# YuvalNirkin/hyperseg

Measured on AMD Instinct MI355X. Metric: frames/sec @ bs=1 HyperSeg-M 1024x512, higher is better.
Workload: dtype f32 storage and accumulation; level-4 inverted residual products as 3-term f16 splits (f32-class: 1.3e-7 of sum|a||b|; exact_f32 beside it)

## Files before the change

hyperseg_amd/_hip.py:

```python
import ctypes as C
import os

import torch

_LIB_PATH = os.environ.get('HS_HIP_LIB') or os.path.join(os.path.dirname(os.path.abspath(__file__)), 'lib',
                                                         'libhyperseg_hip.so')

ACT_NONE, ACT_RELU, ACT_RELU6, ACT_SWISH = 0, 1, 2, 3
PAD_MODES = {'zeros': 0, 'reflect': 1, 'replicate': 2, 'circular': 3}
PREV_NONE, PREV_SAME, PREV_BILINEAR = 0, 1, 2

_STATUS = {-1: 'bad argument', -2: 'feature map does not tile into the weight grid (H % fh or W % fw != 0)',
           -3: 'unsupported shape', -4: 'tile does not fit the LDS'}


class HipLibraryError(RuntimeError):
    pass


class StageInputC(C.Structure):
    _fields_ = [('skip', C.c_void_p), ('prev', C.c_void_p),
                ('batch', C.c_int32), ('H', C.c_int32), ('W', C.c_int32),
                ('c_skip', C.c_int32), ('c_prev', C.c_int32),
                ('Hp', C.c_int32), ('Wp', C.c_int32),
# ... 113 lines not shown
        'hs_patch_conv_plain_bwd_w': ([i32, vp, vp, i32, i32, i32, i32, i32, i32, i32, i32, i32, i32, i32, vp, i64, vp], C.c_int),
        'hs_depthwise_conv_fwd': ([vp, i32, i32, i32, i32, vp, i32, i32, i32, i32, i32, i32, vp, vp, i32, vp, vp, vp, vp, vp], C.c_int),
        'hs_pointwise_conv_fwd': ([vp, i32, i32, i32, vp, i32, vp, vp, vp, i32, vp, vp, vp], C.c_int),
        'hs_affine_act_fwd': ([vp, i32, i32, i32, vp, vp, i32, vp, vp, vp], C.c_int),
        'hs_patch_conv_bn_fwd': ([i32, vp, vp, vp, vp, vp, vp, C.c_float, C.c_float, i32, vp, vp, vp, vp, i64, i32, i32, i32, i32, i32, i32, i32, vp, vp], C.c_int),
        'hs_patch_conv_bn_bwd_w': ([i32, vp, vp, vp, vp, vp, vp, i32, i32, i32, i32, i32, i32, i32, i32, vp, i64, vp], C.c_int),
        'hs_bootstrap_mean_of_batch_fwd': ([vp, i32, i32, i32, C.c_float, vp, vp, vp, vp], C.c_int),
        'hs_bootstrap_mean_of_batch_bwd': ([vp, i32, i32, vp, vp, vp, vp], C.c_int),
        'hs_adam_blocks': ([vp, i32], C.c_int64),
        'hs_adam_step': ([vp, vp, vp, vp, vp, i32, vp, C.c_float, C.c_double, C.c_double, C.c_float, C.c_float, i32, i32, vp, vp], C.c_int),
        'hs_depthwise_pool_blocks': ([i32, i32], C.c_int),
        'hs_depthwise_conv_se_fwd': ([vp, i32, i32, i32, i32, vp, i32, i32, i32, i32, i32, i32, vp, vp, i32, vp, vp, vp, C.POINTER(SeTailC), vp], C.c_int),
        'hs_mbconv_expand_dw_se_fwd': ([vp, i32, i32, i32, i32, vp, i32, vp, vp, vp, i32, i32, i32, i32, i32, i32, vp, vp, vp, C.POINTER(SeTailC), vp], C.c_int),
        'hs_se_tail_workspace': ([i32, i32, i32, i32, i64], C.c_int64),
        'hs_se_tail_tails': ([i32, i32, i32, i64], C.c_int),
        'hs_mbconv_se_workgroups': ([i32, i32, i32, i32, i32, i32], C.c_int64),
        'hs_stem_conv_fwd': ([vp, i32, i32, i32, i32, vp, i32, i32, i32, i32, i32, vp, vp, vp, vp], C.c_int),
        'hs_mbconv_tiles': ([i32, i32, i32, i32], C.c_int),
        'hs_stem_dw_fwd': ([vp, i32, i32, i32, vp, i32, vp, vp, i32, i32, i32, i32, vp, i32, i32, i32, vp, vp, vp, vp, vp], C.c_int),
        'hs_mbconv_expand_dw_fwd': ([vp, i32, i32, i32, i32, vp, i32, vp, vp, vp, i32, i32, i32, i32, i32, i32, vp, vp, vp, vp, vp], C.c_int),
        'hs_se_gate_fwd': ([vp, i32, i32, i32, C.c_float, vp, vp, i32, vp, vp, vp, vp, vp, i32, vp, vp, vp], C.c_int),
        'hs_gemm_split_kp': ([i32], C.c_int),
        'hs_gemm_split_fwd': ([vp, vp, vp, vp, vp, i32, vp, vp, i32, i32, i32, i32, i32, vp], C.c_int),
        'hs_gemm_split_conv2x2_fwd': ([vp, vp, vp, vp, i32, vp, vp, i32, i32, i32, i32, i32, i32, vp], C.c_int),
        'hs_gemm_split_up2_fwd': ([vp, vp, vp, vp, i32, vp, i32, i32, i32, i32, i32, i32, vp], C.c_int),
        'hs_pooled_shift_fwd': ([vp, i32, C.c_float, vp, vp, vp, i32, i32, vp], C.c_int),
    }
    for name, (argtypes, restype) in sig.items():
        fn = getattr(lib, name)
        fn.argtypes, fn.restype = argtypes, restype
    if lib.hs_version() != 1:
        raise HipLibraryError(f'ABI mismatch: library reports version {lib.hs_version()}, binding expects 1')
    return lib


lib = _load()
EXPORTS = ['hs_version', 'hs_build_info', 'hs_signal2weights_fwd', 'hs_signal2weights_multi_fwd', 'hs_s2w_pack_floats', 'hs_s2w_pack_fwd', 'hs_bank_pack_fwd', 'hs_bn_fold_fwd',
           'hs_patch_conv_fwd', 'hs_patch_conv_s2w_fwd', 'hs_k1_chain_workspace', 'hs_k1_chain_fwd', 'hs_decoder_chain_workspace', 'hs_decoder_chain_fwd', 'hs_meta_conv_fwd', 'hs_meta_conv_bwd', 'hs_patch_conv_gen_fwd', 'hs_patch_ir_fwd', 'hs_patch_ir_v0_fwd', 'hs_patch_ir_v0_ws_fwd', 'hs_patch_ir_v0_workspace', 'hs_patch_ir_route', 'hs_ir_tile_map', 'hs_upsample_bilinear_fwd', 'hs_upsample_argmax_fwd',
           'hs_stage_input_fwd', 'hs_depthwise_conv_fwd', 'hs_depthwise_pool_blocks', 'hs_stem_conv_fwd', 'hs_stem_dw_fwd', 'hs_mbconv_tiles', 'hs_mbconv_expand_dw_fwd', 'hs_se_gate_fwd', 'hs_depthwise_conv_se_fwd', 'hs_mbconv_expand_dw_se_fwd', 'hs_se_tail_workspace', 'hs_se_tail_tails', 'hs_mbconv_se_workgroups', 'hs_pointwise_conv_fwd', 'hs_affine_act_fwd', 'hs_gemm_split_kp', 'hs_gemm_split_fwd', 'hs_gemm_split_conv2x2_fwd', 'hs_gemm_split_up2_fwd', 'hs_pooled_shift_fwd', 'hs_patch_conv_bwd_input',
           'hs_patch_conv_bwd_weight', 'hs_halo_tiles_fwd', 'hs_halo_tiles_bwd', 'hs_tile_interior_fwd', 'hs_tile_interior_bwd', 'hs_dw_tiles_fwd', 'hs_dw_tiles_bwd_in', 'hs_dw_tiles_bwd_w',
           'hs_s2w_train_fwd', 'hs_s2w_train_workspace', 'hs_s2w_train_bwd', 'hs_cross_entropy_fwd', 'hs_cross_entropy_bwd', 'hs_cross_entropy_typed_fwd', 'hs_cross_entropy_typed_bwd', 'hs_bootstrapped_ce_fwd', 'hs_bootstrapped_ce_bwd', 'hs_bootstrap_mean_workspace', 'hs_bootstrap_mean_fwd', 'hs_bootstrap_mean_bwd', 'hs_bootstrap_mean_batched_fwd', 'hs_bootstrap_mean_batched_bwd', 'hs_bn_train_workspace', 'hs_bn_train_stats_fwd', 'hs_dw_tiles_bn_fwd', 'hs_dw_tiles_bn_bwd_w', 'hs_patch_conv_bn_fwd', 'hs_patch_conv_bn_bwd_w', 'hs_adam_blocks', 'hs_adam_step', 'hs_bootstrap_mean_of_batch_fwd', 'hs_bootstrap_mean_of_batch_bwd', 'hs_upsample_bilinear_bwd', 'hs_upsample_bilinear_typed_bwd', 'hs_upsample_bilinear_bf16_fwd', 'hs_stage_input_typed_fwd', 'hs_bank_unpack_fwd', 'hs_bn_act_train_fwd',
           'hs_bn_act_train_bwd', 'hs_dw_tiles_bn_bwd_in_partials', 'hs_dw_tiles_bn_bwd_in', 'hs_bn_act_train_bwd_apply', 'hs_patch_conv_plain_fwd', 'hs_patch_conv_plain_bwd_in', 'hs_patch_conv_plain_bwd_w']


def check(status, what):
    if status == 0:
        return
    if status < 0:
        raise HipLibraryError(f'{what}: {_STATUS.get(status, status)}')
    raise HipLibraryError(f'{what}: HIP launch failed with hipError_t {status}')


def dev_ptr(t, name='tensor', dtype=torch.float32):
    if t is None:
        return None
    if not isinstance(t, torch.Tensor):
        raise TypeError(f'{name} must be a torch.Tensor')
    if not t.is_cuda:
        raise HipLibraryError(f'{name} is on {t.device}: the HyperSeg decoder path runs on an MI355X only '
                              '(hyperseg_amd has no CPU fallback)')
    if t.dtype != dtype:
        raise HipLibraryError(f'{name} must be {dtype}, got {t.dtype}')
# ... 25 lines not shown
```

hyperseg_amd/csrc/hs_gemm_split.hip:

```cpp
#include "hs_common.h"
#include <type_traits>

namespace hs {

using half8 = __attribute__((ext_vector_type(8))) _Float16;
using gs_f32x4 = __attribute__((ext_vector_type(4))) float;

__device__ __forceinline__ int gs_exp_of(float m) { return min(max(__float_as_int(m) >> 23, 27), 254); }
__device__ __forceinline__ float gs_scale_of(int eb) { return __int_as_float((268 - eb) << 23); }
__device__ __forceinline__ float gs_inv_scale_of(int eb) { return __int_as_float((eb - 14) << 23); }

struct GemmSplitArgs {
    const _Float16* __restrict__ wf;
    const float* __restrict__ w_inv;
    const float* __restrict__ gate; const float* __restrict__ x;
    const float* shift;
    const float* residual;
    float* y;
    int M, K, KST, N, act;
    int conv_wo;
    float* pool_partial;
    int up2_wo;
};

#ifndef HS_GS_NARROW_MAX_WG
#define HS_GS_NARROW_MAX_WG 128
#endif

#ifndef HS_GS_TALL_MIN_WG
#define HS_GS_TALL_MIN_WG 257
#endif

template <int KS, int NWV, bool FAST, int NS, int MT, int NCH, bool PATCH>
__global__ __launch_bounds__(64 * NWV)
void gemm_split_kernel(GemmSplitArgs a) {
    extern __shared__ __attribute__((aligned(16))) float gs_red[];
    constexpr int nthr = 64 * NWV, nwv = NWV;
    constexpr int NP = 16 * NS, NR = 16 * MT, NE = NR * NP;
    const int tid = threadIdx.x, lane = tid & 63, wave = tid >> 6;
    const int lrow = lane & 15, kg = lane >> 4;
    const int n0 = blockIdx.x * NP, r0 = blockIdx.y * MT, b = blockIdx.z;
    const float* __restrict__ xb = a.x + (size_t)b * a.K * a.N;
    const float* __restrict__ gb = a.gate ? a.gate + (size_t)b * a.K : nullptr;
    float* yb = a.y + (size_t)b * a.M * a.N * (a.up2_wo > 0 ? 4 : 1);
    const float* rb = a.residual ? a.residual + (size_t)b * a.M * a.N : nullptr;
    const int rt_max = (a.M + 15) >> 4;

    using gs_f32x2 = __attribute__((ext_vector_type(2))) float;
    const int ncol0 = min(n0 + NS * lrow, a.N - 1), ncol1 = min(n0 + NS * lrow + 1, a.N - 1);
    float xv[NCH][NS][KS][8];
    if constexpr (PATCH) {
        const int oy = ncol0 / a.conv_wo, ox = ncol0 - oy * a.conv_wo;
        const float* __restrict__ win = xb + (size_t)(2 * oy) * (2 * a.conv_wo) + 2 * ox;
        const int cmax = (a.K >> 2) - 1;
#pragma unroll
        for (int c = 0; c < NCH; ++c)
#pragma unroll
            for (int s = 0; s < KS; ++s)
#pragma unroll
                for (int q = 0; q < 4; ++q) {
                    const int ch = min((((wave * NCH + c) * KS + s) * 32 + 8 * kg) / 4 + (q >> 1), cmax);
                    const float* src = win + (size_t)ch * (4 * a.N) + (q & 1) * (2 * a.conv_wo);
                    if constexpr (NS == 1) {
                        const gs_f32x2 v = *reinterpret_cast<const gs_f32x2*>(src);
                        xv[c][0][s][2 * q] = v[0]; xv[c][0][s][2 * q + 1] = v[1];
                    } else {
                        const gs_f32x4 v = *reinterpret_cast<const gs_f32x4*>(src);
                        xv[c][0][s][2 * q] = v[0]; xv[c][0][s][2 * q + 1] = v[1];
                        xv[c][1][s][2 * q] = v[2]; xv[c][1][s][2 * q + 1] = v[3];
                    }
                }
    } else {
#pragma unroll
        for (int c = 0; c < NCH; ++c)
#pragma unroll
            for (int s = 0; s < KS; ++s)
#pragma unroll
                for (int j = 0; j < 8; ++j) {
                    const int k = ((wave * NCH + c) * KS + s) * 32 + 8 * kg + j;
                    const int kc = min(k, a.K - 1);
                    if constexpr (NS == 1) {
                        xv[c][0][s][j] = xb[(size_t)kc * a.N + ncol0];
                    } else if constexpr (FAST) {
                        const gs_f32x2 v = *reinterpret_cast<const gs_f32x2*>(xb + (size_t)kc * a.N + ncol0);
                        xv[c][0][s][j] = v[0]; xv[c][1][s][j] = v[1];
                    } else {
                        xv[c][0][s][j] = xb[(size_t)kc * a.N + ncol0]; xv[c][1][s][j] = xb[(size_t)kc * a.N + ncol1];
                    }
                }
    }
    constexpr int NG = PATCH ? 1 : NCH;
    float gv[NG][KS][8];
    if constexpr (!PATCH) {
#pragma unroll
        for (int c = 0; c < NCH; ++c)
#pragma unroll
            for (int s = 0; s < KS; ++s) {
                const int k0 = ((wave * NCH + c) * KS + s) * 32 + 8 * kg;
                if constexpr (FAST) {
                    const float* gp = gb ? gb + min(k0, a.K - 8) : a.w_inv;
                    const gs_f32x4 g0 = *reinterpret_cast<const gs_f32x4*>(gp), g1 = *reinterpret_cast<const gs_f32x4*>(gp + 4);
#pragma unroll
                    for (int j = 0; j < 4; ++j) { gv[c][s][j] = g0[j]; gv[c][s][4 + j] = g1[j]; }
                } else {
#pragma unroll
                    for (int j = 0; j < 8; ++j) gv[c][s][j] = gb ? gb[min(k0 + j, a.K - 1)] : 1.0f;
                }
            }
    }
    half8 ah[2][KS], al[2][KS];
    auto load_a = [&](int q) {
        const int rt = min(r0 + q % MT, rt_max - 1);
#pragma unroll
        for (int s = 0; s < KS; ++s) {
            const _Float16* blk = a.wf + ((size_t)(rt * a.KST + (wave * NCH + q / MT) * KS + s) * 2) * 512 + lane * 8;
            ah[q & 1][s] = *reinterpret_cast<const half8*>(blk);
            al[q & 1][s] = *reinterpret_cast<const half8*>(blk + 512);
        }
    };
    load_a(0);
    constexpr int TE = (NE + nthr - 1) / nthr;
    float wi[TE], sh[TE], yo[TE];
    auto load_tail = [&]() {
#pragma unroll
        for (int i = 0; i < TE; ++i) {
            const int e = min(tid + i * nthr, NE - 1);
            const int row = min(16 * r0 + e / NP, a.M - 1), col = min(n0 + (e & (NP - 1)), a.N - 1);
            wi[i] = a.w_inv[min(16 * r0 + e / NP, 16 * rt_max - 1)];
            sh[i] = a.shift ? a.shift[row] : 0.0f;
            yo[i] = rb ? rb[(size_t)row * a.N + col] : 0.0f;
        }
    };
    constexpr bool LATE_TAIL = KS * NCH >= 3;
    if constexpr (!LATE_TAIL) load_tail();
    __builtin_amdgcn_sched_barrier(0);

    gs_f32x4 tot[MT][NS];
#pragma unroll
    for (int c = 0; c < NCH; ++c) {
        float invb[NS];
        half8 bh[NS][KS], bl[NS][KS];
#pragma unroll
        for (int t = 0; t < NS; ++t) {
            unsigned mx = 0;
#pragma unroll
            for (int s = 0; s < KS; ++s) {
                const int k0 = ((wave * NCH + c) * KS + s) * 32 + 8 * kg;
#pragma unroll
                for (int j = 0; j < 8; ++j) {
                    const float mk = (FAST || PATCH ? k0 : k0 + j) < a.K ? 1.0f : 0.0f;
                    float g = mk;
                    if constexpr (!PATCH) g = gb ? gv[c][s][j] * mk : mk;
                    xv[c][t][s][j] *= g;
                    mx = max(mx, __float_as_uint(xv[c][t][s][j]) & 0x7fffffffu);
                }
            }
            {
                auto r16 = __builtin_amdgcn_permlane16_swap(mx, mx, false, false);
                mx = max(r16[0], r16[1]);
                auto r32 = __builtin_amdgcn_permlane32_swap(mx, mx, false, false);
                mx = max(r32[0], r32[1]);
            }
            const int eb = gs_exp_of(__uint_as_float(mx));
            const float sc = gs_scale_of(eb);
            invb[t] = gs_inv_scale_of(eb);
#pragma unroll
            for (int s = 0; s < KS; ++s) {
                if constexpr (FAST || PATCH) {
                    unsigned hh[4], ll[4];
#pragma unroll
                    for (int j = 0; j < 4; ++j) {
                        asm("v_fma_mixlo_f16 %0, %2, %4, 0\n\t"
                            "v_fma_mixhi_f16 %0, %3, %4, 0\n\t"
                            "v_fma_mixlo_f16 %1, %2, %4, -%0 op_sel_hi:[0,0,1]\n\t"
                            "v_fma_mixhi_f16 %1, %3, %4, -%0 op_sel:[0,0,1] op_sel_hi:[0,0,1]"
// ... 114 lines not shown

static bool gemm_split_plan(int K, int& nwv, int& ks, int& nch) {
    const int steps = (K + 31) / 32;
    nwv = 2;
    while (nwv < 8 && nwv < steps) nwv *= 2;
    const int per = (steps + nwv - 1) / nwv;
    nch = per > 5 ? 2 : 1;
    ks = (steps + nwv * nch - 1) / (nwv * nch);
    return ks <= 5;
}

}

using namespace hs;

extern "C" int hs_gemm_split_kp(int32_t c_in) {
    int nwv, ks, nch;
    if (c_in <= 0 || !gemm_split_plan(c_in, nwv, ks, nch)) return HS_ERR_UNSUPPORTED;
    return nwv * nch * ks * 32;
}

static int launch_gemm_split_plain(const void* w_frag, const float* w_inv, const float* gate, const float* x, const float* shift,
                                   int32_t act, const float* residual, float* y, int32_t batch, int32_t c_out, int32_t c_in,
                                   int32_t kp, int32_t pixels, int up2_wo, void* stream) {
    if (!w_frag || !w_inv || !x || !y || batch <= 0 || c_out <= 0 || c_in <= 0 || pixels <= 0) return HS_ERR_BAD_ARG;
    if (act < 0 || act > 3) return HS_ERR_BAD_ARG;
    int nwv, ks, nch;
    if (!gemm_split_plan(c_in, nwv, ks, nch)) return HS_ERR_UNSUPPORTED;
    if (kp != nwv * nch * ks * 32 || (ks > 1 && nwv != 8)) return HS_ERR_BAD_ARG;
    if (batch > 65535 || (c_out + 31) / 32 > 65535) return HS_ERR_UNSUPPORTED;
    GemmSplitArgs a{(const _Float16*)w_frag, w_inv, gate, x, shift, residual, y, c_out, c_in, kp / 32, pixels, act, 0, nullptr, up2_wo};
    dim3 grid((pixels + 31) / 32, ((c_out + 15) / 16 + 1) / 2, batch);
    const size_t wgs = (size_t)grid.x * grid.y * grid.z;
    const bool narrow = wgs <= HS_GS_NARROW_MAX_WG && pixels > 16;
    const bool tall = wgs >= HS_GS_TALL_MIN_WG && c_out > 32;
    if (narrow) grid.x = (pixels + 15) / 16;
    if (tall) grid.y = ((c_out + 15) / 16 + 3) / 4;
    const size_t lds = (size_t)nwv * (narrow ? 512 : tall ? 2048 : 1024) * sizeof(float);
    hipStream_t s = (hipStream_t)stream;
    const bool fast = (c_in & 7) == 0 && (pixels & 1) == 0 && c_in >= 8;
#define HS_GS_(KSV, NWV, F) do { \
        if (narrow) hipLaunchKernelGGL((gemm_split_kernel<KSV, NWV, F, 1, 2, 1, false>), grid, dim3(64 * NWV), lds, s, a); \
        else if (tall) hipLaunchKernelGGL((gemm_split_kernel<KSV, NWV, F, 2, 4, 1, false>), grid, dim3(64 * NWV), lds, s, a); \
        else hipLaunchKernelGGL((gemm_split_kernel<KSV, NWV, F, 2, 2, 1, false>), grid, dim3(64 * NWV), lds, s, a); } while (0)
#define HS_GS(KSV, NWV) do { if (fast) HS_GS_(KSV, NWV, true); else HS_GS_(KSV, NWV, false); } while (0)
    if (nch == 2) {
        if (!fast || up2_wo > 0) return HS_ERR_UNSUPPORTED;
        grid.x = (pixels + 15) / 16; grid.y = ((c_out + 15) / 16 + 1) / 2;
        const size_t lds2 = (size_t)8 * 512 * sizeof(float);
#define HS_GS2(KSV) hipLaunchKernelGGL((gemm_split_kernel<KSV, 8, true, 1, 2, 2, false>), grid, dim3(512), lds2, s, a)
        switch (ks) { case 3: HS_GS2(3); break; case 4: HS_GS2(4); break; case 5: HS_GS2(5); break; default: return HS_ERR_UNSUPPORTED; }
#undef HS_GS2
        return launch_status();
    }
    switch (ks) {
        case 1: if (nwv == 2) HS_GS(1, 2); else if (nwv == 4) HS_GS(1, 4); else HS_GS(1, 8); break;
        case 2: HS_GS(2, 8); break;
        case 3: HS_GS(3, 8); break;
        case 4: HS_GS(4, 8); break;
        default: HS_GS(5, 8); break;
    }
#undef HS_GS
#undef HS_GS_
    return launch_status();
}

extern "C" int hs_gemm_split_fwd(const void* w_frag, const float* w_inv, const float* gate, const float* x,
                                 const float* shift, int32_t act, const float* residual, float* y,
                                 int32_t batch, int32_t c_out, int32_t c_in, int32_t kp, int32_t pixels, void* stream) {
    return launch_gemm_split_plain(w_frag, w_inv, gate, x, shift, act, residual, y, batch, c_out, c_in, kp, pixels, 0, stream);
}

extern "C" int hs_gemm_split_up2_fwd(const void* w_frag, const float* w_inv, const float* x, const float* shift, int32_t act,
                                     float* y, int32_t batch, int32_t c_out, int32_t c_in, int32_t kp, int32_t Ho, int32_t Wo,
                                     void* stream) {
    if (Ho <= 0 || Wo <= 0 || (((size_t)y) & 7) != 0) return HS_ERR_BAD_ARG;
    return launch_gemm_split_plain(w_frag, w_inv, nullptr, x, shift, act, nullptr, y, batch, c_out, c_in, kp, Ho * Wo, Wo, stream);
}

extern "C" int hs_pooled_shift_fwd(const float* partial, int32_t nblk, float inv_pixels, const float* wb, const float* shift,
                                   float* shift_out, int32_t rows, int32_t channels, void* stream) {
    if (!partial || !wb || !shift || !shift_out || nblk <= 0 || rows <= 0 || channels <= 0) return HS_ERR_BAD_ARG;
    if (channels > 8192) return HS_ERR_UNSUPPORTED;
    hipLaunchKernelGGL(pooled_shift_kernel, dim3((rows + 15) / 16), dim3(256), (size_t)channels * sizeof(float), (hipStream_t)stream,
                       partial, nblk, inv_pixels, wb, shift, shift_out, rows, channels);
    return launch_status();
}

extern "C" int hs_gemm_split_conv2x2_fwd(const void* w_frag, const float* w_inv, const float* x, const float* shift, int32_t act,
                                         float* y, float* pool_partial, int32_t batch, int32_t c_out, int32_t c_in, int32_t kp,
                                         int32_t Ho, int32_t Wo, void* stream) {
    if (!w_frag || !w_inv || !x || !y || batch <= 0 || c_out <= 0 || c_in <= 0 || Ho <= 0 || Wo <= 0) return HS_ERR_BAD_ARG;
    if (act < 0 || act > 3) return HS_ERR_BAD_ARG;
// ... 26 lines not shown
```

hyperseg_amd/functional.py:

```python
import ctypes as C
import functools
import os
import threading

import torch

from . import _hip
from ._hip import ACT_NONE, ACT_RELU, ACT_RELU6, PAD_MODES

BN_EPS_DEFAULT = 1e-5
S2W_TRAIN_MAX_LAYERS = 8
USE_SIDE_STREAM = os.environ.get('HS_SIDE_STREAM', '0') == '1'
PIPELINE_BANKS = os.environ.get('HS_SIDE_STREAM', '0') == '2'
COSCHEDULE_BANKS = os.environ.get('HS_COSCHEDULE_BANKS', '0') == '1'


def _round_up(n, m):
    return (n + m - 1) // m * m


def _device_of(a):
    if isinstance(a, torch.Tensor):
        return a.device
    if isinstance(a, (StageInput, BankRef, SignalRef)):
# ... 910 lines not shown
    m, k = w.shape
    kp = _hip.lib.hs_gemm_split_kp(k) if k <= max_k else -1
    if kp < 0:
        return None
    if row_scale is not None:
        w = w * row_scale.detach().float()[:, None]
    eb = (w.abs().amax(1).contiguous().view(torch.int32) >> 23).clamp(27, 254)
    one = torch.ones(m, device=w.device)
    ws = w * torch.ldexp(one, 141 - eb)[:, None]
    hi = ws.half()
    lo = (ws - hi.float()).half()
    rt = -(-m // 16)
    pad = (0, kp - k, 0, 16 * rt - m)
    hi, lo = torch.nn.functional.pad(hi, pad), torch.nn.functional.pad(lo, pad)
    inv = torch.nn.functional.pad(torch.ldexp(one, eb - 141), (0, 16 * rt - m), value=1.0)

    def fragment_order(t):
        return t.view(rt, 16, kp // 32, 4, 8).permute(0, 2, 3, 1, 4)
    frag = torch.stack([fragment_order(hi), fragment_order(lo)], dim=2).contiguous()
    return SplitWeights(frag, inv.contiguous(), m, k, kp)


@_on_operand_device
def gemm_split(sw, x, gate=None, shift=None, act=ACT_NONE, residual=None, out=None):
    b, cin, h, w = x.shape
    if cin != sw.c_in:
        raise ValueError(f'input has {cin} channels, the weight {sw.c_in}')
    shape = (b, sw.c_out, h, w)
    if out is None:
        out = torch.empty(shape, device=x.device, dtype=torch.float32)
    elif tuple(out.shape) != shape:
        raise ValueError(f'out has shape {tuple(out.shape)}, expected {shape}')
    if residual is not None and tuple(residual.shape) != shape:
        raise ValueError(f'residual has shape {tuple(residual.shape)}, expected {shape}')
    if gate is not None and tuple(gate.shape) != (b, cin):
        raise ValueError(f'gate has shape {tuple(gate.shape)}, expected {(b, cin)}')
    if shift is not None and shift.numel() != sw.c_out:
        raise ValueError(f'shift has {shift.numel()} entries, expected {sw.c_out}')
    st = _hip.lib.hs_gemm_split_fwd(_hip.dev_ptr(sw.frag, 'w_frag', torch.float16), _hip.dev_ptr(sw.inv, 'w_inv'),
                                    _hip.dev_ptr(gate, 'gate') if gate is not None else None, _hip.dev_ptr(x, 'x'),
                                    _hip.dev_ptr(shift, 'shift') if shift is not None else None, int(act),
                                    _hip.dev_ptr(residual, 'residual') if residual is not None else None,
                                    _hip.dev_ptr(out, 'out'), b, sw.c_out, cin, sw.kp, h * w, _hip.stream_ptr())
    _hip.check(st, 'hs_gemm_split_fwd')
    return out


@_on_operand_device
def gemm_split_conv2x2(sw, x, shift=None, act=ACT_NONE, out=None, pool_partial=None):
    b, cin, h, w = x.shape
    if 4 * cin != sw.c_in:
        raise ValueError(f'input has {cin} channels, the weight {sw.c_in} / 4')
    if h % 2 or w % 4:
        raise ValueError(f'map {h}x{w}: height must be even and width a multiple of 4')
    shape = (b, sw.c_out, h // 2, w // 2)
    if out is None:
        out = torch.empty(shape, device=x.device, dtype=torch.float32)
    elif tuple(out.shape) != shape:
        raise ValueError(f'out has shape {tuple(out.shape)}, expected {shape}')
    if shift is not None and shift.numel() != sw.c_out:
        raise ValueError(f'shift has {shift.numel()} entries, expected {sw.c_out}')
    nblk = -(-(h // 2) * (w // 2) // 16)
    if pool_partial is not None and tuple(pool_partial.shape) != (b, sw.c_out, nblk):
        raise ValueError(f'pool_partial has shape {tuple(pool_partial.shape)}, expected {(b, sw.c_out, nblk)}')
    st = _hip.lib.hs_gemm_split_conv2x2_fwd(_hip.dev_ptr(sw.frag, 'w_frag', torch.float16), _hip.dev_ptr(sw.inv, 'w_inv'),
                                            _hip.dev_ptr(x, 'x'), _hip.dev_ptr(shift, 'shift') if shift is not None else None,
                                            int(act), _hip.dev_ptr(out, 'out'),
# ... 113 lines not shown
```

hyperseg_amd/utils/inference.py:

```python
import contextlib
import os

import torch
import torch.nn as nn


@torch.no_grad()
def _fold(conv, bn):
    scale = bn.weight / torch.sqrt(bn.running_var + bn.eps)
    shift = bn.bias - bn.running_mean * scale
    conv.weight.mul_(scale.view(-1, 1, 1, 1))
    if conv.bias is not None:
        conv.bias.mul_(scale).add_(shift)
    else:
        conv.bias = nn.Parameter(shift.clone())


def _fold_pairs(module, pairs):
    n = 0
    for conv_name, bn_name in pairs:
        conv, bn = getattr(module, conv_name, None), getattr(module, bn_name, None)
        if isinstance(conv, nn.Conv2d) and isinstance(bn, nn.BatchNorm2d) and not bn.training:
            _fold(conv, bn)
            setattr(module, bn_name, nn.Identity())
# ... 1 lines not shown
    return n


def _fold_sequential(seq):
    n = 0
    mods = list(seq)
    for i in range(len(mods) - 1):
        if isinstance(mods[i], nn.Conv2d) and isinstance(mods[i + 1], nn.BatchNorm2d) and not mods[i + 1].training:
            _fold(mods[i], mods[i + 1])
            seq[i + 1] = nn.Identity()
            n += 1
    return n


def _bn_affine(bn):
    with torch.no_grad():
        scale = bn.weight / torch.sqrt(bn.running_var + bn.eps)
        shift = bn.bias - bn.running_mean * scale
    return scale.detach().clone(), shift.detach().clone()


SPLIT_GEMM_MAX_K = int(os.environ.get('HS_SPLIT_GEMM_MAX_K', '1280'))
STEM_DW = os.environ.get('HS_STEM_DW', '1') != '0'
FUSE_EXPAND_MIN_PIXELS = int(os.environ.get('HS_FUSE_EXPAND_MIN_PIXELS', '2048'))
FUSE_EXPAND_MAX_CIN = int(os.environ.get('HS_FUSE_EXPAND_MAX_CIN', '40'))


LEAN_MFMA_MAX_CIN = int(os.environ.get('HS_LEAN_MFMA_MAX_CIN', '16'))
PW_MFMA_MAX_CIN = int(os.environ.get('HS_PW_MFMA_MAX_CIN', '96'))
PW_MFMA_MIN_PIXELS = int(os.environ.get('HS_PW_MFMA_MIN_PIXELS', '8192'))
GEMM_LT_MIN_PIXELS = int(os.environ.get('HS_GEMM_LT_MIN_PIXELS', '16384'))


@contextlib.contextmanager
def gemm_library(pixels, batch=1):
    want = os.environ.get('HS_BLAS') or ('cublaslt' if (pixels >= GEMM_LT_MIN_PIXELS or batch > 1) else 'cublas')
    prev = torch.backends.cuda.preferred_blas_library()
    torch.backends.cuda.preferred_blas_library(want)
    try:
        yield
    finally:
        torch.backends.cuda.preferred_blas_library(prev)


class FusedPointwise(nn.Module):

# ... 164 lines not shown
                                      blk._depthwise_conv.weight, self.stride, self.pad_t, self.pad_l, (ho, wo),
                                      self.scale, self.shift, pool=True, se=se)
        else:
            in_scale = in_shift = None
            if self.expand is not None:
                if lean and not self.expand.uses_mfma(x):
                    in_scale, in_shift = self.expand.scale, self.expand.shift
                    x = self.expand.raw(x)
                else:
                    x = self.expand(x)
            out = HF.depthwise_conv_bn_act(x, blk._depthwise_conv.weight, self.stride, self.pad_t, self.pad_l,
                                           (ho, wo), self.scale, self.shift, act=3, pool=True,
                                           in_scale=in_scale, in_shift=in_shift, se=se)
        y, pooled, gated = out if se is not None else (out[0], out[1], False)

        def se_gate(**fold):
            if gated and not fold:
                return pooled
            return HF.se_gate(pooled, b, ho * wo, red.weight, red.bias, self._exp_t, exp.bias, **fold)
        skip = inputs.contiguous() if self.skip else None
        if lean_gemm:
            sw = proj.split_weights(True, y.device) if proj.split_gemm else None
            if sw is not None:
                gate = se_gate()
                if self.defer_shift:
                    if skip is None:
                        return HF.gemm_split(sw, y, gate=gate)
                    return HF.gemm_split(sw, y, gate=gate, residual=skip, out=skip)
                return HF.gemm_split(sw, y, gate=gate, shift=proj.shift, residual=skip)
            wp = se_gate(w_proj=proj.conv.weight, out_scale=proj.scale)
            cmid = y.shape[1]
            with gemm_library(ho * wo, b):
                if b == 1:
                    w2d, y2d = wp.view(-1, cmid), y.view(cmid, ho * wo)
                    if self.defer_shift:
                        if skip is None:
                            return torch.mm(w2d, y2d).view(1, -1, ho, wo)
                        skip.view(-1, ho * wo).addmm_(w2d, y2d)
                        return skip
                    out = torch.mm(w2d, y2d).view(1, -1, ho, wo)
                else:
                    w3d, y3d = wp.view(b, -1, cmid), y.view(b, cmid, ho * wo)
                    if self.defer_shift:
                        if skip is None:
                            return torch.bmm(w3d, y3d).view(b, -1, ho, wo)
                        skip.view(b, -1, ho * wo).baddbmm_(w3d, y3d)
                        return skip
                    out = torch.bmm(w3d, y3d).view(b, -1, ho, wo)
            return HF.affine_act_(out, None, proj.shift, 0, skip)
        return proj(y, gate=se_gate(), residual=skip)


# ... 292 lines not shown
```

include/hyperseg_hip.h:

```cpp
#ifndef HYPERSEG_HIP_H
#define HYPERSEG_HIP_H

#include <stdint.h>

#ifdef __cplusplus
extern "C" {
#endif

#define HS_ABI_VERSION 1

typedef enum {
    HS_OK = 0,
    HS_ERR_BAD_ARG = -1,
    HS_ERR_NOT_DIVISIBLE = -2,
    HS_ERR_UNSUPPORTED = -3,
    HS_ERR_LDS = -4
} hs_status;

typedef enum { HS_ACT_NONE = 0, HS_ACT_RELU = 1, HS_ACT_RELU6 = 2, HS_ACT_SWISH = 3 } hs_act;
typedef enum { HS_PAD_ZEROS = 0, HS_PAD_REFLECT = 1, HS_PAD_REPLICATE = 2, HS_PAD_CIRCULAR = 3 } hs_pad_mode;
typedef enum { HS_PREV_NONE = 0, HS_PREV_SAME = 1, HS_PREV_BILINEAR = 2 } hs_prev_mode;

typedef struct {
    const float* skip;
// ... 174 lines not shown
int hs_mbconv_expand_dw_fwd(const float* x, int32_t batch, int32_t c_in, int32_t H, int32_t W,
                            const float* w_expand, int32_t c_mid, const float* scale0, const float* shift0,
                            const float* w_dw, int32_t k, int32_t stride, int32_t pad_t, int32_t pad_l,
                            int32_t Ho, int32_t Wo, const float* scale1, const float* shift1, float* y,
                            float* pool_partial, void* stream);
int64_t hs_mbconv_se_workgroups(int32_t batch, int32_t c_mid, int32_t k, int32_t stride, int32_t Ho, int32_t Wo);
int hs_mbconv_expand_dw_se_fwd(const float* x, int32_t batch, int32_t c_in, int32_t H, int32_t W,
                               const float* w_expand, int32_t c_mid, const float* scale0, const float* shift0,
                               const float* w_dw, int32_t k, int32_t stride, int32_t pad_t, int32_t pad_l,
                               int32_t Ho, int32_t Wo, const float* scale1, const float* shift1, float* y,
                               const hs_se_tail* se, void* stream);

int hs_pointwise_conv_fwd(const float* x, int32_t batch, int32_t c_in, int32_t pixels, const float* w, int32_t c_out,
                          const float* gate, const float* scale, const float* shift, int32_t act, const float* residual,
                          float* y, void* stream);

int hs_affine_act_fwd(const float* x, int32_t batch, int32_t channels, int32_t pixels, const float* scale,
                      const float* shift, int32_t act, const float* residual, float* y, void* stream);

int hs_gemm_split_kp(int32_t c_in);
int hs_gemm_split_fwd(const void* w_frag, const float* w_inv, const float* gate, const float* x, const float* shift,
                      int32_t act, const float* residual, float* y, int32_t batch, int32_t c_out, int32_t c_in, int32_t kp,
                      int32_t pixels, void* stream);
int hs_gemm_split_conv2x2_fwd(const void* w_frag, const float* w_inv, const float* x, const float* shift, int32_t act, float* y,
                              float* pool_partial, int32_t batch, int32_t c_out, int32_t c_in, int32_t kp, int32_t Ho,
                              int32_t Wo, void* stream);
int hs_gemm_split_up2_fwd(const void* w_frag, const float* w_inv, const float* x, const float* shift, int32_t act, float* y,
                          int32_t batch, int32_t c_out, int32_t c_in, int32_t kp, int32_t Ho, int32_t Wo, void* stream);
int hs_pooled_shift_fwd(const float* partial, int32_t nblk, float inv_pixels, const float* wb, const float* shift,
                        float* shift_out, int32_t rows, int32_t channels, void* stream);

int hs_halo_tiles_fwd(int32_t dtype, const void* x, int32_t batch, int32_t channels, int32_t H, int32_t W, int32_t fh, int32_t fw,
                      void* tiled, int32_t patch_major, void* stream);
int hs_halo_tiles_bwd(int32_t dtype, const void* dtiled, int32_t batch, int32_t channels, int32_t H, int32_t W, int32_t fh, int32_t fw,
                      void* dx, int32_t patch_major, void* stream);
int hs_tile_interior_fwd(int32_t dtype, const void* tiled, int32_t batch, int32_t channels, int32_t H, int32_t W, int32_t fh,
                         int32_t fw, void* y, void* stream);
int hs_tile_interior_bwd(int32_t dtype, const void* dy, int32_t batch, int32_t channels, int32_t H, int32_t W, int32_t fh, int32_t fw,
                         void* dtiled, void* stream);
int hs_dw_tiles_fwd(int32_t dtype, const void* tiled, const float* bank, int64_t ld, int32_t batch, int32_t channels, int32_t H, int32_t W,
                    int32_t fh, int32_t fw, void* y, int32_t patch_major, void* stream);
int hs_dw_tiles_bwd_in(int32_t dtype, const void* dy, const float* bank, int64_t ld, int32_t batch, int32_t channels, int32_t H, int32_t W,
                       int32_t fh, int32_t fw, void* dtiled, int32_t patch_major, void* stream);
int hs_dw_tiles_bwd_w(int32_t dtype, const void* tiled, const void* dy, int32_t batch, int32_t channels, int32_t H, int32_t W, int32_t fh,
                      int32_t fw, float* dbank, int64_t ld, int32_t patch_major, void* stream);
int64_t hs_bootstrap_mean_workspace(void);
// ... 91 lines not shown
```

Before: 1352.

## Fuse SE gate computation into split-GEMM projection kernel prologue

Adds an SE variant of the split-f16 GEMM kernel. Each workgroup reduces the pooled partials, runs the squeeze-excite reduce/expand MLP and sigmoid in LDS, and applies the gate to its input slice before the projection GEMM. This removes the separate SE gate launch and its global round trip for batch-1 inference. In exchange every workgroup recomputes the small SE MLP redundantly and needs extra LDS and registers, which may lower occupancy.

```diff
diff --git a/hyperseg_amd/_hip.py b/hyperseg_amd/_hip.py
--- a/hyperseg_amd/_hip.py
+++ b/hyperseg_amd/_hip.py
@@ -159,6 +159,7 @@
         'hs_se_gate_fwd': ([vp, i32, i32, i32, C.c_float, vp, vp, i32, vp, vp, vp, vp, vp, i32, vp, vp, vp], C.c_int),
         'hs_gemm_split_kp': ([i32], C.c_int),
         'hs_gemm_split_fwd': ([vp, vp, vp, vp, vp, i32, vp, vp, i32, i32, i32, i32, i32, vp], C.c_int),
+        'hs_gemm_split_se_fwd': ([vp, vp, vp, vp, i32, vp, vp, i32, i32, i32, i32, i32, vp, i32, C.c_float, vp, vp, vp, vp, i32, vp], C.c_int),
         'hs_gemm_split_conv2x2_fwd': ([vp, vp, vp, vp, i32, vp, vp, i32, i32, i32, i32, i32, i32, vp], C.c_int),
         'hs_gemm_split_up2_fwd': ([vp, vp, vp, vp, i32, vp, i32, i32, i32, i32, i32, i32, vp], C.c_int),
         'hs_pooled_shift_fwd': ([vp, i32, C.c_float, vp, vp, vp, i32, i32, vp], C.c_int),
@@ -174,7 +175,7 @@
 lib = _load()
 EXPORTS = ['hs_version', 'hs_build_info', 'hs_signal2weights_fwd', 'hs_signal2weights_multi_fwd', 'hs_s2w_pack_floats', 'hs_s2w_pack_fwd', 'hs_bank_pack_fwd', 'hs_bn_fold_fwd',
            'hs_patch_conv_fwd', 'hs_patch_conv_s2w_fwd', 'hs_k1_chain_workspace', 'hs_k1_chain_fwd', 'hs_decoder_chain_workspace', 'hs_decoder_chain_fwd', 'hs_meta_conv_fwd', 'hs_meta_conv_bwd', 'hs_patch_conv_gen_fwd', 'hs_patch_ir_fwd', 'hs_patch_ir_v0_fwd', 'hs_patch_ir_v0_ws_fwd', 'hs_patch_ir_v0_workspace', 'hs_patch_ir_route', 'hs_ir_tile_map', 'hs_upsample_bilinear_fwd', 'hs_upsample_argmax_fwd',
-           'hs_stage_input_fwd', 'hs_depthwise_conv_fwd', 'hs_depthwise_pool_blocks', 'hs_stem_conv_fwd', 'hs_stem_dw_fwd', 'hs_mbconv_tiles', 'hs_mbconv_expand_dw_fwd', 'hs_se_gate_fwd', 'hs_depthwise_conv_se_fwd', 'hs_mbconv_expand_dw_se_fwd', 'hs_se_tail_workspace', 'hs_se_tail_tails', 'hs_mbconv_se_workgroups', 'hs_pointwise_conv_fwd', 'hs_affine_act_fwd', 'hs_gemm_split_kp', 'hs_gemm_split_fwd', 'hs_gemm_split_conv2x2_fwd', 'hs_gemm_split_up2_fwd', 'hs_pooled_shift_fwd', 'hs_patch_conv_bwd_input',
+           'hs_stage_input_fwd', 'hs_depthwise_conv_fwd', 'hs_depthwise_pool_blocks', 'hs_stem_conv_fwd', 'hs_stem_dw_fwd', 'hs_mbconv_tiles', 'hs_mbconv_expand_dw_fwd', 'hs_se_gate_fwd', 'hs_depthwise_conv_se_fwd', 'hs_mbconv_expand_dw_se_fwd', 'hs_se_tail_workspace', 'hs_se_tail_tails', 'hs_mbconv_se_workgroups', 'hs_pointwise_conv_fwd', 'hs_affine_act_fwd', 'hs_gemm_split_kp', 'hs_gemm_split_fwd', 'hs_gemm_split_se_fwd', 'hs_gemm_split_conv2x2_fwd', 'hs_gemm_split_up2_fwd', 'hs_pooled_shift_fwd', 'hs_patch_conv_bwd_input',
            'hs_patch_conv_bwd_weight', 'hs_halo_tiles_fwd', 'hs_halo_tiles_bwd', 'hs_tile_interior_fwd', 'hs_tile_interior_bwd', 'hs_dw_tiles_fwd', 'hs_dw_tiles_bwd_in', 'hs_dw_tiles_bwd_w',
            'hs_s2w_train_fwd', 'hs_s2w_train_workspace', 'hs_s2w_train_bwd', 'hs_cross_entropy_fwd', 'hs_cross_entropy_bwd', 'hs_cross_entropy_typed_fwd', 'hs_cross_entropy_typed_bwd', 'hs_bootstrapped_ce_fwd', 'hs_bootstrapped_ce_bwd', 'hs_bootstrap_mean_workspace', 'hs_bootstrap_mean_fwd', 'hs_bootstrap_mean_bwd', 'hs_bootstrap_mean_batched_fwd', 'hs_bootstrap_mean_batched_bwd', 'hs_bn_train_workspace', 'hs_bn_train_stats_fwd', 'hs_dw_tiles_bn_fwd', 'hs_dw_tiles_bn_bwd_w', 'hs_patch_conv_bn_fwd', 'hs_patch_conv_bn_bwd_w', 'hs_adam_blocks', 'hs_adam_step', 'hs_bootstrap_mean_of_batch_fwd', 'hs_bootstrap_mean_of_batch_bwd', 'hs_upsample_bilinear_bwd', 'hs_upsample_bilinear_typed_bwd', 'hs_upsample_bilinear_bf16_fwd', 'hs_stage_input_typed_fwd', 'hs_bank_unpack_fwd', 'hs_bn_act_train_fwd',
            'hs_bn_act_train_bwd', 'hs_dw_tiles_bn_bwd_in_partials', 'hs_dw_tiles_bn_bwd_in', 'hs_bn_act_train_bwd_apply', 'hs_patch_conv_plain_fwd', 'hs_patch_conv_plain_bwd_in', 'hs_patch_conv_plain_bwd_w']
diff --git a/hyperseg_amd/csrc/hs_gemm_split.hip b/hyperseg_amd/csrc/hs_gemm_split.hip
--- a/hyperseg_amd/csrc/hs_gemm_split.hip
+++ b/hyperseg_amd/csrc/hs_gemm_split.hip
@@ -23,6 +23,18 @@
     int up2_wo;
 };
 
+struct GemmSplitSe {
+    const float* __restrict__ partial;
+    const float* __restrict__ w1;
+    const float* __restrict__ b1;
+    const float* __restrict__ w2t;
+    const float* __restrict__ b2;
+    int nblk, Csq;
+    float inv_hw;
+};
+constexpr int GS_SE_MAX_C = 512, GS_SE_MAX_CSQ = 32, GS_SE_MAX_UNITS = 2048;
+constexpr int GS_SE_LDS_FLOATS = GS_SE_MAX_C + GS_SE_MAX_CSQ + GS_SE_MAX_C + GS_SE_MAX_UNITS + GS_SE_MAX_C;
+
 #ifndef HS_GS_NARROW_MAX_WG
 #define HS_GS_NARROW_MAX_WG 128
 #endif
@@ -31,10 +43,12 @@
 #define HS_GS_TALL_MIN_WG 257
 #endif
 
-template <int KS, int NWV, bool FAST, int NS, int MT, int NCH, bool PATCH>
+template <int KS, int NWV, bool FAST, int NS, int MT, int NCH, bool PATCH, typename... Se>
 __global__ __launch_bounds__(64 * NWV)
-void gemm_split_kernel(GemmSplitArgs a) {
+void gemm_split_kernel(GemmSplitArgs a, Se... se_pack) {
     extern __shared__ __attribute__((aligned(16))) float gs_red[];
+    constexpr bool SE = sizeof...(Se) > 0;
+    static_assert(sizeof...(Se) <= 1 && (std::is_same_v<Se, GemmSplitSe> && ...), "Se: empty or GemmSplitSe");
     constexpr int nthr = 64 * NWV, nwv = NWV;
     constexpr int NP = 16 * NS, NR = 16 * MT, NE = NR * NP;
     const int tid = threadIdx.x, lane = tid & 63, wave = tid >> 6;
@@ -45,6 +59,54 @@
     float* yb = a.y + (size_t)b * a.M * a.N * (a.up2_wo > 0 ? 4 : 1);
     const float* rb = a.residual ? a.residual + (size_t)b * a.M * a.N : nullptr;
     const int rt_max = (a.M + 15) >> 4;
+
+    constexpr int SE_PU = GS_SE_MAX_UNITS / 512, SE_GR = (KS + 1) / 2;
+    float4 se_pv[SE ? SE_PU : 1], se_w1[SE ? 4 : 1][3];
+    float se_b1[SE ? 4 : 1], se_w2[SE ? SE_GR : 1][4][8], se_b2[SE ? SE_GR : 1];
+    int se_qn = 1, se_units = 0, se_jq = 0;
+    int wv = 0;
+    GemmSplitSe se{};
+    if constexpr (SE) {
+        se = (se_pack, ...);
+        wv = __builtin_amdgcn_readfirstlane(wave);
+        static_assert(NWV == 8 && FAST && !PATCH && NCH == 1 && KS <= 2, "SE prologue: the 8-wave FAST form, K <= 512");
+        const int C = a.K, Csq = se.Csq, c4 = C >> 2;
+        const bool vec = (se.nblk & 3) == 0;
+        se_qn = vec ? se.nblk >> 2 : se.nblk;
+        se_units = C * se_qn;
+        const float* __restrict__ pb = se.partial + (size_t)b * C * se.nblk;
+        if (vec) {
+#pragma unroll
+            for (int k = 0; k < SE_PU; ++k) se_pv[k] = reinterpret_cast<const float4*>(pb)[min(tid + 512 * k, se_units - 1)];
+        } else {
+#pragma unroll
+            for (int k = 0; k < SE_PU; ++k) se_pv[k] = make_float4(pb[min(tid + 512 * k, se_units - 1)], 0.0f, 0.0f, 0.0f);
+        }
+#pragma unroll
+        for (int r = 0; r < 4; ++r) {
+            const int j = min(wv + 8 * r, Csq - 1);
+            se_b1[r] = se.b1[j];
+#pragma unroll
+            for (int u = 0; u < 3; ++u) {
+                se_w1[r][u] = make_float4(0.0f, 0.0f, 0.0f, 0.0f);
+                if (wv + 8 * r < Csq && 64 * u < c4)
+                    se_w1[r][u] = reinterpret_cast<const float4*>(se.w1 + (size_t)j * C)[min(lane + 64 * u, c4 - 1)];
+            }
+        }
+        se_jq = (Csq + 3) >> 2;
+#pragma unroll
+        for (int h = 0; h < SE_GR; ++h) {
+            const int cc = min(wv * KS * 32 + lane + 64 * h, C - 1);
+            se_b2[h] = se.b2[cc];
+#pragma unroll
+            for (int p = 0; p < 4; ++p)
+#pragma unroll
+                for (int u = 0; u < 8; ++u) {
+                    se_w2[h][p][u] = 0.0f;
+                    if (u < se_jq) se_w2[h][p][u] = se.w2t[(size_t)min(p * se_jq + u, Csq - 1) * C + cc];
+                }
+        }
+    }
 
     using gs_f32x2 = __attribute__((ext_vector_type(2))) float;
     const int ncol0 = min(n0 + NS * lrow, a.N - 1), ncol1 = min(n0 + NS * lrow + 1, a.N - 1);
@@ -91,7 +153,7 @@
     }
     constexpr int NG = PATCH ? 1 : NCH;
     float gv[NG][KS][8];
-    if constexpr (!PATCH) {
+    if constexpr (!PATCH && !SE) {
 #pragma unroll
         for (int c = 0; c < NCH; ++c)
 #pragma unroll
@@ -135,6 +197,73 @@
     if constexpr (!LATE_TAIL) load_tail();
     __builtin_amdgcn_sched_barrier(0);
 
+    if constexpr (SE) {
+        float* se_gate = gs_red + nwv * NE;
+        float* se_zs = se_gate + GS_SE_MAX_C;
+        float* se_mean = se_zs + GS_SE_MAX_CSQ;
+        float* se_part = se_mean + GS_SE_MAX_C;
+        const int C = a.K, Csq = se.Csq, c4 = C >> 2;
+#pragma unroll
+        for (int k = 0; k < SE_PU; ++k) {
+            const int e = tid + 512 * k;
+            if (e < se_units) {
+                const int ch = e / se_qn;
+                se_part[ch * (se_qn + 1) + (e - ch * se_qn)] = (se_pv[k].x + se_pv[k].y) + (se_pv[k].z + se_pv[k].w);
+            }
+        }
+        __syncthreads();
+        for (int ch = tid; ch < C; ch += 512) {
+            const float* run = se_part + ch * (se_qn + 1);
+            float t = 0.0f;
+            for (int i = 0; i < se_qn; ++i) t += run[i];
+            se_mean[ch] = t * se.inv_hw;
+        }
+        __syncthreads();
+        float4 mv[3];
+#pragma unroll
+        for (int u = 0; u < 3; ++u) {
+            const int k = lane + 64 * u;
+            mv[u] = *reinterpret_cast<const float4*>(se_mean + 4 * min(k, c4 - 1));
+            if (k >= c4) mv[u] = make_float4(0.0f, 0.0f, 0.0f, 0.0f);
+        }
+#pragma unroll
+        for (int r = 0; r < 4; ++r) {
+            if (wv + 8 * r < Csq) {
+                float t = 0.0f;
+#pragma unroll
+                for (int u = 0; u < 3; ++u) {
+                    t = fmaf(se_w1[r][u].x, mv[u].x, t); t = fmaf(se_w1[r][u].y, mv[u].y, t);
+                    t = fmaf(se_w1[r][u].z, mv[u].z, t); t = fmaf(se_w1[r][u].w, mv[u].w, t);
+                }
+                t = wave_sum64(t);
+                if (lane == 0) se_zs[wv + 8 * r] = swishf(t + se_b1[r]);
+            }
+        }
+        __syncthreads();
+#pragma unroll
+        for (int h = 0; h < SE_GR; ++h) {
+            float q[4];
+#pragma unroll
+            for (int p = 0; p < 4; ++p) {
+                const int j0 = p * se_jq, j1 = min(j0 + se_jq, Csq);
+                q[p] = 0.0f;
+#pragma unroll
+                for (int u = 0; u < 8; ++u)
+                    if (j0 + u < j1) q[p] = fmaf(se_w2[h][p][u], se_zs[j0 + u], q[p]);
+            }
+            if (lane + 64 * h < KS * 32)
+                se_gate[wv * KS * 32 + lane + 64 * h] = sigmoidf_fast(((q[0] + q[1]) + (q[2] + q[3])) + se_b2[h]);
+        }
+        __syncthreads();
+#pragma unroll
+        for (int s = 0; s < KS; ++s) {
+            const float* gp = se_gate + (wave * KS + s) * 32 + 8 * kg;
+            const gs_f32x4 g0 = *reinterpret_cast<const gs_f32x4*>(gp), g1 = *reinterpret_cast<const gs_f32x4*>(gp + 4);
+#pragma unroll
+            for (int j = 0; j < 4; ++j) { gv[0][s][j] = g0[j]; gv[0][s][4 + j] = g1[j]; }
+        }
+    }
+
     gs_f32x4 tot[MT][NS];
 #pragma unroll
     for (int c = 0; c < NCH; ++c) {
@@ -150,7 +279,7 @@
                 for (int j = 0; j < 8; ++j) {
                     const float mk = (FAST || PATCH ? k0 : k0 + j) < a.K ? 1.0f : 0.0f;
                     float g = mk;
-                    if constexpr (!PATCH) g = gb ? gv[c][s][j] * mk : mk;
+                    if constexpr (!PATCH) g = (SE || gb) ? gv[c][s][j] * mk : mk;
                     xv[c][t][s][j] *= g;
                     mx = max(mx, __float_as_uint(xv[c][t][s][j]) & 0x7fffffffu);
                 }
@@ -311,7 +440,7 @@
 
 static int launch_gemm_split_plain(const void* w_frag, const float* w_inv, const float* gate, const float* x, const float* shift,
                                    int32_t act, const float* residual, float* y, int32_t batch, int32_t c_out, int32_t c_in,
-                                   int32_t kp, int32_t pixels, int up2_wo, void* stream) {
+                                   int32_t kp, int32_t pixels, int up2_wo, void* stream, const GemmSplitSe* se = nullptr) {
     if (!w_frag || !w_inv || !x || !y || batch <= 0 || c_out <= 0 || c_in <= 0 || pixels <= 0) return HS_ERR_BAD_ARG;
     if (act < 0 || act > 3) return HS_ERR_BAD_ARG;
     int nwv, ks, nch;
@@ -328,6 +457,21 @@
     const size_t lds = (size_t)nwv * (narrow ? 512 : tall ? 2048 : 1024) * sizeof(float);
     hipStream_t s = (hipStream_t)stream;
     const bool fast = (c_in & 7) == 0 && (pixels & 1) == 0 && c_in >= 8;
+    if (se) {
+        if (!fast || nwv != 8 || nch != 1 || ks > 2 || up2_wo > 0 || gate) return HS_ERR_UNSUPPORTED;
+        const size_t lds_se = lds + (size_t)GS_SE_LDS_FLOATS * sizeof(float);
+#define HS_GSE_(KSV) do { \
+        if (narrow) hipLaunchKernelGGL((gemm_split_kernel<KSV, 8, true, 1, 2, 1, false, GemmSplitSe>), grid, dim3(512), lds_se, s, a, *se); \
+        else if (tall) {  \
+            static std::atomic<unsigned long long> done{0}; \
+            const int e = allow_full_lds((const void*)gemm_split_kernel<KSV, 8, true, 2, 4, 1, false, GemmSplitSe>, done); \
+            if (e != HS_OK) return e; \
+            hipLaunchKernelGGL((gemm_split_kernel<KSV, 8, true, 2, 4, 1, false, GemmSplitSe>), grid, dim3(512), lds_se, s, a, *se); } \
+        else hipLaunchKernelGGL((gemm_split_kernel<KSV, 8, true, 2, 2, 1, false, GemmSplitSe>), grid, dim3(512), lds_se, s, a, *se); } while (0)
+        if (ks == 1) HS_GSE_(1); else HS_GSE_(2);
+#undef HS_GSE_
+        return launch_status();
+    }
 #define HS_GS_(KSV, NWV, F) do { \
         if (narrow) hipLaunchKernelGGL((gemm_split_kernel<KSV, NWV, F, 1, 2, 1, false>), grid, dim3(64 * NWV), lds, s, a); \
         else if (tall) hipLaunchKernelGGL((gemm_split_kernel<KSV, NWV, F, 2, 4, 1, false>), grid, dim3(64 * NWV), lds, s, a); \
@@ -358,6 +502,20 @@
                                  const float* shift, int32_t act, const float* residual, float* y,
                                  int32_t batch, int32_t c_out, int32_t c_in, int32_t kp, int32_t pixels, void* stream) {
     return launch_gemm_split_plain(w_frag, w_inv, gate, x, shift, act, residual, y, batch, c_out, c_in, kp, pixels, 0, stream);
+}
+
+extern "C" int hs_gemm_split_se_fwd(const void* w_frag, const float* w_inv, const float* x, const float* shift, int32_t act,
+                                    const float* residual, float* y, int32_t batch, int32_t c_out, int32_t c_in, int32_t kp,
+                                    int32_t pixels, const float* partial, int32_t nblk, float inv_hw, const float* w_reduce,
+                                    const float* b_reduce, const float* w_expand, const float* b_expand, int32_t c_squeezed,
+                                    void* stream) {
+    if (!partial || !w_reduce || !b_reduce || !w_expand || !b_expand || nblk <= 0 || c_squeezed <= 0) return HS_ERR_BAD_ARG;
+    const long units = (long)c_in * ((nblk & 3) == 0 ? nblk >> 2 : nblk);
+    if (c_in <= 0 || c_in > GS_SE_MAX_C || (c_in & 7) != 0 || c_squeezed > GS_SE_MAX_CSQ || units > GS_SE_MAX_UNITS) return HS_ERR_UNSUPPORTED;
+    if ((nblk & 3) == 0 && (((size_t)partial) & 15) != 0) return HS_ERR_BAD_ARG;
+    if ((((size_t)w_reduce) & 15) != 0) return HS_ERR_BAD_ARG;
+    const GemmSplitSe se{partial, w_reduce, b_reduce, w_expand, b_expand, nblk, c_squeezed, inv_hw};
+    return launch_gemm_split_plain(w_frag, w_inv, nullptr, x, shift, act, residual, y, batch, c_out, c_in, kp, pixels, 0, stream, &se);
 }
 
 extern "C" int hs_gemm_split_up2_fwd(const void* w_frag, const float* w_inv, const float* x, const float* shift, int32_t act,
diff --git a/hyperseg_amd/functional.py b/hyperseg_amd/functional.py
--- a/hyperseg_amd/functional.py
+++ b/hyperseg_amd/functional.py
@@ -956,7 +956,9 @@
 
 
 @_on_operand_device
-def gemm_split(sw, x, gate=None, shift=None, act=ACT_NONE, residual=None, out=None):
+def gemm_split(sw, x, gate=None, shift=None, act=ACT_NONE, residual=None, out=None, se=None):
+    if se is not None:
+        return _gemm_split_se(sw, x, se, shift, act, residual, out, gate)
     b, cin, h, w = x.shape
     if cin != sw.c_in:
         raise ValueError(f'input has {cin} channels, the weight {sw.c_in}')
@@ -977,6 +979,43 @@
                                     _hip.dev_ptr(residual, 'residual') if residual is not None else None,
                                     _hip.dev_ptr(out, 'out'), b, sw.c_out, cin, sw.kp, h * w, _hip.stream_ptr())
     _hip.check(st, 'hs_gemm_split_fwd')
+    return out
+
+
+def _gemm_split_se(sw, x, se, shift, act, residual, out, gate):
+    if gate is not None:
+        raise ValueError('gate= and se= are exclusive')
+    partial, hw, w_reduce, b_reduce, w_expand_t, b_expand = se
+    b, cin, h, w = x.shape
+    if cin != sw.c_in:
+        raise ValueError(f'input has {cin} channels, the weight {sw.c_in}')
+    csq = w_reduce.shape[0]
+    if partial.dim() != 2 or partial.shape[0] != b * cin:
+        raise ValueError(f'partial has shape {tuple(partial.shape)}, expected ({b * cin}, nblk)')
+    if tuple(w_reduce.shape) != (csq, cin) or tuple(w_expand_t.shape) != (csq, cin):
+        raise ValueError(f'w_reduce {tuple(w_reduce.shape)} / w_expand_t {tuple(w_expand_t.shape)}: expected ({csq}, {cin}) each')
+    if b_reduce.numel() != csq or b_expand.numel() != cin:
+        raise ValueError(f'b_reduce has {b_reduce.numel()} entries, b_expand {b_expand.numel()}: expected {csq} and {cin}')
+    shape = (b, sw.c_out, h, w)
+    if out is None:
+        out = torch.empty(shape, device=x.device, dtype=torch.float32)
+    elif tuple(out.shape) != shape:
+        raise ValueError(f'out has shape {tuple(out.shape)}, expected {shape}')
+    if residual is not None and tuple(residual.shape) != shape:
+        raise ValueError(f'residual has shape {tuple(residual.shape)}, expected {shape}')
+    if shift is not None and shift.numel() != sw.c_out:
+        raise ValueError(f'shift has {shift.numel()} entries, expected {sw.c_out}')
+    st = _hip.lib.hs_gemm_split_se_fwd(_hip.dev_ptr(sw.frag, 'w_frag', torch.float16), _hip.dev_ptr(sw.inv, 'w_inv'),
+                                       _hip.dev_ptr(x, 'x'), _hip.dev_ptr(shift, 'shift') if shift is not None else None, int(act),
+                                       _hip.dev_ptr(residual, 'residual') if residual is not None else None,
+                                       _hip.dev_ptr(out, 'out'), b, sw.c_out, cin, sw.kp, h * w,
+                                       _hip.dev_ptr(partial, 'partial'), partial.shape[1], 1.0 / float(hw),
+                                       _hip.dev_ptr(w_reduce, 'w_reduce'), _hip.dev_ptr(b_reduce, 'b_reduce'),
+                                       _hip.dev_ptr(w_expand_t, 'w_expand'), _hip.dev_ptr(b_expand, 'b_expand'), csq,
+                                       _hip.stream_ptr())
+    if st == -3:
+        return None
+    _hip.check(st, 'hs_gemm_split_se_fwd')
     return out
 
 
diff --git a/hyperseg_amd/utils/inference.py b/hyperseg_amd/utils/inference.py
--- a/hyperseg_amd/utils/inference.py
+++ b/hyperseg_amd/utils/inference.py
@@ -47,6 +47,8 @@
 
 SPLIT_GEMM_MAX_K = int(os.environ.get('HS_SPLIT_GEMM_MAX_K', '1280'))
 STEM_DW = os.environ.get('HS_STEM_DW', '1') != '0'
+SE_IN_GEMM = os.environ.get('HS_SE_IN_GEMM', '1') != '0'
+SE_IN_GEMM_MAX_BATCH = int(os.environ.get('HS_SE_IN_GEMM_MAX_BATCH', '1'))
 FUSE_EXPAND_MIN_PIXELS = int(os.environ.get('HS_FUSE_EXPAND_MIN_PIXELS', '2048'))
 FUSE_EXPAND_MAX_CIN = int(os.environ.get('HS_FUSE_EXPAND_MAX_CIN', '40'))
 
@@ -257,12 +259,15 @@
         if lean_gemm:
             sw = proj.split_weights(True, y.device) if proj.split_gemm else None
             if sw is not None:
-                gate = se_gate()
                 if self.defer_shift:
-                    if skip is None:
-                        return HF.gemm_split(sw, y, gate=gate)
-                    return HF.gemm_split(sw, y, gate=gate, residual=skip, out=skip)
-                return HF.gemm_split(sw, y, gate=gate, shift=proj.shift, residual=skip)
+                    epi = dict(residual=skip, out=skip) if skip is not None else {}
+                else:
+                    epi = dict(shift=proj.shift, residual=skip)
+                if SE_IN_GEMM and not gated and b <= SE_IN_GEMM_MAX_BATCH and y.is_cuda:
+                    out = HF.gemm_split(sw, y, se=(pooled, ho * wo, self._red_w, red.bias, self._exp_t, exp.bias), **epi)
+                    if out is not None:
+                        return out
+                return HF.gemm_split(sw, y, gate=se_gate(), **epi)
             wp = se_gate(w_proj=proj.conv.weight, out_scale=proj.scale)
             cmid = y.shape[1]
             with gemm_library(ho * wo, b):
diff --git a/include/hyperseg_hip.h b/include/hyperseg_hip.h
--- a/include/hyperseg_hip.h
+++ b/include/hyperseg_hip.h
@@ -220,6 +220,10 @@
 int hs_gemm_split_fwd(const void* w_frag, const float* w_inv, const float* gate, const float* x, const float* shift,
                       int32_t act, const float* residual, float* y, int32_t batch, int32_t c_out, int32_t c_in, int32_t kp,
                       int32_t pixels, void* stream);
+int hs_gemm_split_se_fwd(const void* w_frag, const float* w_inv, const float* x, const float* shift, int32_t act,
+                         const float* residual, float* y, int32_t batch, int32_t c_out, int32_t c_in, int32_t kp, int32_t pixels,
+                         const float* partial, int32_t nblk, float inv_hw, const float* w_reduce, const float* b_reduce,
+                         const float* w_expand, const float* b_expand, int32_t c_squeezed, void* stream);
 int hs_gemm_split_conv2x2_fwd(const void* w_frag, const float* w_inv, const float* x, const float* shift, int32_t act, float* y,
                               float* pool_partial, int32_t batch, int32_t c_out, int32_t c_in, int32_t kp, int32_t Ho,
                               int32_t Wo, void* stream);
```

Result: faster. 1371, median of 6 (+1.4%).
